# nyrahealth/CrisperWhisper

Hardware: AMD Instinct MI355X
Metric: aligned words/s (RTF alongside), CrisperWhisper large-v3 geometry, 30 s chunks, full mel->encoder->decoder->DTW->words path (higher is better)
Workload: dtype bf16

## Files before the change

### crisperwhisper_amd/csrc/engine.hip

```cpp
#include <hip/hip_runtime.h>
#include <stdarg.h>
#include <stdlib.h>
#include <string.h>
#include <set>
#include <string>
#include <vector>
#include <functional>
#include <algorithm>

#include "../../include/crisperwhisper.h"
#include "kernels.h"

static thread_local char g_err[512] = "";

#define KD(c, fn, ...) ((c)->f16 ? cw_f16::fn(__VA_ARGS__) : cw_bf16::fn(__VA_ARGS__))

#define CW_MAX_DEC_STAGES 24
enum DecStageKind { DST_OTHER = 0, DST_QKV_SELF, DST_QKV, DST_SELF_ATTN, DST_O_PROJ, DST_STACK, DST_STACK_CROSS, DST_CROSS_Q, DST_CROSS_ATTN,
                    DST_CROSS_O, DST_FC1, DST_FC2, DST_MLP_PAIR, DST_MLP_CHAIN, DST_N };
static const char* const kDecStageName[DST_N] = {
    "other (A/B path)", "LayerNorm + q/k/v projection + self-attention (qkv_self_kernel)", "LayerNorm + q/k/v projection + cache append",
    "self-attention", "self-attention out-projection", "fused out-projection + cross-query stage (gemv_stack_kernel)",
    "fused stage + cross-attention (dec_layer_a_kernel)", "LayerNorm + cross-attention query projection", "cross-attention",
    "cross-attention out-projection (combines the key-split partials)", "LayerNorm + fc1 + GELU", "fc2", "fc1 + fc2 (mlp_pair_kernel)",
// ... 2575 lines not shown
                CWCHK(c, dmalloc(c, &L.wqkv8, (size_t)3 * D * D, false)); CWCHK(c, dmalloc(c, &L.sqkv, (size_t)3 * D * 4));
                CWCHK(c, dmalloc(c, &L.w18, (size_t)F * D, false)); CWCHK(c, dmalloc(c, &L.s1, (size_t)F * 4));
                CWCHK(c, dmalloc(c, &L.w28, (size_t)D * F, false)); CWCHK(c, dmalloc(c, &L.s2, (size_t)D * 4));
            }
            for (auto& L : c->dec) { CWCHK(c, dmalloc(c, &L.wkv_c8, (size_t)2 * D * D, false)); CWCHK(c, dmalloc(c, &L.skv_c, (size_t)2 * D * 4)); }
        }
        CWCHK(c, enc8_quantise(c));
        c->enc8 = true;
        c->enc8_mask = value >= 16 ? ((value - 16) & 15) : 15;
        c->nb_encoded = 0;
        return CW_OK;
    }
#ifndef CW_EXPERIMENTS
    if ((!strcmp(name, "rows_ln") || !strcmp(name, "skinny")) && value != 0)
        return fail(c, CW_ERR_INVALID, "option %s selects a measured-and-rejected kernel variant that is not in this build (make EXTRA=-DCW_EXPERIMENTS)", name);
#endif
    if (!strcmp(name, "test_epoch_forwards")) {
        c->forwards_since_reset = (long long)value;
        return CW_OK;
    }
    if (!strcmp(name, "handoff_fail_pos")) {
        c->fail_pos = value;
        for (auto& ge : c->step_graph) if (ge) { hipGraphExecDestroy(ge); ge = nullptr; }
        return CW_OK;
    }
    if (!strcmp(name, "rows_ln")) {
        c->rows_ln_enabled = value != 0;
        for (auto& ge : c->step_graph) if (ge) { hipGraphExecDestroy(ge); ge = nullptr; }
        return CW_OK;
    }
    if (!strcmp(name, "skinny")) {
        c->skinny_mode = value;
        for (auto& ge : c->step_graph) if (ge) { hipGraphExecDestroy(ge); ge = nullptr; }
        return CW_OK;
    }
    return fail(c, CW_ERR_INVALID, "unknown option %s", name);
}

int32_t cw_has_experiments(void) {
#ifdef CW_EXPERIMENTS
    return 1;
#else
    return 0;
#endif
}

static int g_test_cross_fp8 = 0;
int32_t cw_test_set_option(const char* name, int32_t value) {
    if (!strcmp(name, "cross_test_fp8")) { g_test_cross_fp8 = value; return CW_OK; }
    if (!strcmp(name, "gemm256_min_tiles")) { cw_bf16::cw_gemm_set_256_min_tiles(value); cw_f16::cw_gemm_set_256_min_tiles(value); return CW_OK; }
    if (!strcmp(name, "beam_topk_1block")) { cw_bf16::cw_beam_topk_set_1block(value); cw_f16::cw_beam_topk_set_1block(value); return CW_OK; }
    if (!strcmp(name, "gemm_pp")) { cw_bf16::cw_gemm_set_pp(value); cw_f16::cw_gemm_set_pp(value); return CW_OK; }
    if (!strcmp(name, "gemm_8ph")) { cw_bf16::cw_gemm_set_8ph(value); cw_f16::cw_gemm_set_8ph(value); return CW_OK; }
    if (!strcmp(name, "gemm_gm")) {
#ifndef CW_EXPERIMENTS
        return CW_ERR_INVALID;
#endif
        cw_bf16::cw_gemm_set_gm(value); cw_f16::cw_gemm_set_gm(value); return CW_OK;
    }
    if (!strcmp(name, "gemv_loop")) { cw_bf16::cw_gemv_set_loop(value); cw_f16::cw_gemv_set_loop(value); return CW_OK; }
    if (!strcmp(name, "mt_variant")) { cw_bf16::cw_gemv_set_mt_variant(value); cw_f16::cw_gemv_set_mt_variant(value); return CW_OK; }
    if (!strcmp(name, "comb_rowgroups")) { cw_bf16::cw_gemv_set_comb_rowgroups(value); cw_f16::cw_gemv_set_comb_rowgroups(value); return CW_OK; }
    if (!strcmp(name, "gemm_w128")) { cw_bf16::cw_gemm_set_w128(value); cw_f16::cw_gemm_set_w128(value); return CW_OK; }
    if (!strcmp(name, "cross_valu")) { cw_bf16::cw_cross_set_valu(value); cw_f16::cw_cross_set_valu(value); return CW_OK; }
    if (!strcmp(name, "cross_per_row")) { cw_bf16::cw_cross_set_per_row(value); cw_f16::cw_cross_set_per_row(value); return CW_OK; }
    return CW_ERR_INVALID;
}

int32_t cw_test_gemm(cw_ctx* c, int32_t M, int32_t N, int32_t K, const float* A, const float* W, const float* bias,
                     int32_t gelu, float* out) {
    void *dA = nullptr, *dW = nullptr, *dO = nullptr; float* dB = nullptr;
    const size_t e = c->esz;
    HIPCHK(c, hipMalloc(&dA, (size_t)M * K * e)); HIPCHK(c, hipMalloc(&dW, (size_t)N * K * e));
    HIPCHK(c, hipMalloc(&dO, (size_t)M * N * e)); HIPCHK(c, hipMalloc((void**)&dB, (size_t)N * 4));
    CWCHK(c, upload_T(c, dA, 0, A, (size_t)M * K)); CWCHK(c, upload_T(c, dW, 0, W, (size_t)N * K));
    if (bias) HIPCHK(c, hipMemcpy(dB, bias, (size_t)N * 4, hipMemcpyHostToDevice));
    AParams ap{dA, K, 0, 0, 0, 0, nullptr, nullptr};
    EpiParams ep = epi0(); ep.out = dO; ep.bias = bias ? dB : nullptr; ep.ldo = N;
    int r = KD(c, cw_launch_gemm, c->bf16, gelu ? EPI_GELU : EPI_STORE, ap, dW, M, N, K, ep, c->st);
    if (r == CW_OK) { hipError_t er = hipStreamSynchronize(c->st); if (er != hipSuccess) r = fail(c, CW_ERR_HIP, "test_gemm: %s", hipGetErrorString(er)); }
    if (const int reps = cw_sw::cw_switches().test_gemm_reps) {
        hipEvent_t e0, e1;
        if (r == CW_OK && reps > 0 && hipEventCreate(&e0) == hipSuccess && hipEventCreate(&e1) == hipSuccess) {
            hipEventRecord(e0, c->st);
            for (int i = 0; i < reps && r == CW_OK; ++i) r = KD(c, cw_launch_gemm, c->bf16, gelu ? EPI_GELU : EPI_STORE, ap, dW, M, N, K, ep, c->st);
            hipEventRecord(e1, c->st);
            hipEventSynchronize(e1);
            float ms = 0.f;
            hipEventElapsedTime(&ms, e0, e1);
            const double us = 1e3 * ms / reps;
            fprintf(stderr, "[cw_test_gemm] M=%d N=%d K=%d gelu=%d: %.2f us/launch, %.1f TFLOP/s\n", M, N, K, gelu, us, 2.0 * M * N * K / us * 1e-6);
            hipEventDestroy(e0); hipEventDestroy(e1);
        }
    }
    if (r == CW_OK) r = download_T(c, dO, 0, out, (size_t)M * N);
    hipFree(dA); hipFree(dW); hipFree(dO); hipFree(dB);
    return r;
}

int32_t cw_test_prefill_gemm(cw_ctx* c, int32_t mode, int32_t M, int32_t N, int32_t K, const float* A, const float* W,
                             const float* bias, float* out) {
    if (!c->bf16) return fail(c, CW_ERR_INVALID, "test_prefill_gemm: 16-bit engines only");
    if ((mode != PF_STORE && mode != PF_RESID && mode != PF_GELU) || M < 1 || N < 16 || N % 16 || K < 32 || K % 32)
        return fail(c, CW_ERR_INVALID, "test_prefill_gemm: bad arguments");
    void *dA = nullptr, *dW = nullptr, *dWp = nullptr, *dO = nullptr; float* dB = nullptr;
    const size_t e = c->esz;
// ... 885 lines not shown
```

### crisperwhisper_amd/csrc/gemm.hip

```cpp
#include "common.h"
#include "kernels.h"
#include <stdlib.h>
#include <mutex>
#include "gemm_tiles.h"

namespace CW_NS {

#define BM 128
#define BN 128
#define LDS_STRIDE 72

typedef __attribute__((ext_vector_type(4))) unsigned int u32x4_t;

__device__ inline f32x4_t mfma16(bf16x8_t a, bf16x8_t b, f32x4_t c) { return cw_mfma_16x16x32(a, b, c); }

template <typename TA>
__device__ inline const TA* a_row_ptr(const AParams& ap, int m, int M, int k0) {
    if (m >= M) return nullptr;
    if (ap.amode == 0) return (const TA*)ap.A + (size_t)m * ap.lda + k0;
    int b = m / ap.T_out, t = m - b * ap.T_out;
    int tap = k0 / ap.C_in, c0 = k0 - tap * ap.C_in;
    int t_in = t * ap.stride + tap - 1;
    if (t_in < 0 || t_in >= ap.row_valid[b]) return nullptr;
    return (const TA*)ap.A + ((size_t)(ap.row_off[b] + t_in)) * ap.C_in + c0;
// ... 419 lines not shown
            asm volatile("s_waitcnt vmcnt(0)" ::: "memory");
            __builtin_amdgcn_s_barrier();
        }
        __builtin_amdgcn_s_barrier();
    } else {
        __builtin_amdgcn_s_barrier();
        for (int t = 0; t < nk; ++t) {
            read_frags(t & 1);
            if (t + 1 < nk) issue((t + 1) * BK, (t + 1) & 1);
            asm volatile("s_waitcnt vmcnt(0) lgkmcnt(0)" ::: "memory");
            __builtin_amdgcn_s_barrier();
            mfmas();
            __builtin_amdgcn_s_barrier();
        }
    }

    const bool vec_ok = (EPI == EPI_HEADS || (ep.ldo & 3) == 0);
    if (m0 + BM2 <= M && vec_ok) {
        int cols[4];
#pragma unroll
        for (int j = 0; j < 4; ++j) cols[j] = n0 + wn * 64 + j * 16 + g * 4;
#pragma unroll
        for (int h = 0; h < 2; ++h) {
            int rows[4];
#pragma unroll
            for (int i = 0; i < 4; ++i) rows[i] = m0 + wm * 128 + (h * 4 + i) * 16 + l15;
            epi_tile_interior<bf16_t, EPI>(ep, rows, cols, *(const f32x4_t(*)[4][4])&acc[h * 4]);
        }
        return;
    }
#pragma unroll
    for (int i = 0; i < 8; ++i) {
        int m = m0 + wm * 128 + i * 16 + l15;
        if (m >= M) continue;
#pragma unroll
        for (int j = 0; j < 4; ++j) {
            int n = n0 + wn * 64 + j * 16 + g * 4;
            if (vec_ok) {
                epi_store4<bf16_t, EPI>(ep, m, n, acc[i][j][0], acc[i][j][1], acc[i][j][2], acc[i][j][3]);
            } else {
#pragma unroll
                for (int r = 0; r < 4; ++r) epi_store1<bf16_t, EPI>(ep, m, n + r, acc[i][j][r]);
            }
        }
    }
}

#endif

#ifdef CW_EXPERIMENTS
__constant__ int c_gemm_gm = 8;
#endif

template <int EPI>
__global__ __launch_bounds__(512) void gemm_bf16_8ph_kernel(const bf16_t* __restrict__ A, int lda,
                                                            const bf16_t* __restrict__ W, int M, int N, int K,
                                                            EpiParams ep, int tiles_n) {
    extern __shared__ __attribute__((aligned(16))) unsigned char gsm4[];
    const int tid = threadIdx.x, lane = tid & 63;
    const int wave = __builtin_amdgcn_readfirstlane(tid >> 6);
    const int wr = wave >> 2, wn = wave & 3;
    const int l15 = lane & 15, g = lane >> 4;
#ifdef CW_EXPERIMENTS
    const int gm_ = c_gemm_gm;
    const int tile = gm_ < 0 ? (int)blockIdx.x : xcd_remap(blockIdx.x, gridDim.x);
    int mt_, nt_;
    grouped_tile(tile, gridDim.x / tiles_n, tiles_n, mt_, nt_, gm_ < 0 ? -gm_ : gm_);
#else
    const int tile = xcd_remap(blockIdx.x, gridDim.x);
    int mt_, nt_;
    grouped_tile(tile, gridDim.x / tiles_n, tiles_n, mt_, nt_);
#endif
    const int m0 = mt_ * BM2, n0 = nt_ * BN2;

    const int lrow = lane >> 3;
    const int csrc = ((lane & 7) ^ lrow) * 8;
    const __amdgpu_buffer_rsrc_t ra = __builtin_amdgcn_make_buffer_rsrc((void*)A, (short)0, 0x7fffffff, 0x00020000);
    const __amdgpu_buffer_rsrc_t rw = __builtin_amdgcn_make_buffer_rsrc((void*)W, (short)0, 0x7fffffff, 0x00020000);
    int va[2][2];
#pragma unroll
    for (int h = 0; h < 2; ++h)
#pragma unroll
        for (int q = 0; q < 2; ++q) va[h][q] = (min(m0 + h * 128 + wave * 16 + q * 8 + lrow, M - 1) * lda + csrc) * 2;
    const int vw = ((n0 + wave * 16 + lrow) * K + csrc) * 2;
    auto issue_a = [&](int k0, int buf, int h) {
#ifdef CW_8PH_NO_DMA
        return;
#endif
        unsigned char* base = gsm4 + buf * 65536 + (h * 128 + wave * 16) * 128;
#pragma unroll
        for (int q = 0; q < 2; ++q)
            __builtin_amdgcn_raw_ptr_buffer_load_lds(ra, (__attribute__((address_space(3))) void*)(base + q * 1024), 16, va[h][q], k0 * 2, 0, 0);
    };
    auto issue_w = [&](int k0, int buf, int h) {
#ifdef CW_8PH_NO_DMA
        return;
#endif
        unsigned char* base = gsm4 + buf * 65536 + 32768 + (h * 128 + wave * 16) * 128;
#pragma unroll
        for (int q = 0; q < 2; ++q)
            __builtin_amdgcn_raw_ptr_buffer_load_lds(rw, (__attribute__((address_space(3))) void*)(base + q * 1024), 16, vw,
                                                     (k0 + (h * 128 + q * 8) * K) * 2, 0, 0);
    };
    const int sw = l15 & 7;
    const int aoff = (wr * 64 + l15) * 128, woff = 32768 + (wn * 32 + l15) * 128;
    bf16x8_t fa[2][4], fw[2][2][2];
    auto read_a = [&](int buf, int h) {
#ifdef CW_8PH_NO_READS
        if (buf >= 0) return;
#endif
        const unsigned char* sb = gsm4 + buf * 65536 + aoff + h * 16384;
#pragma unroll
        for (int kk = 0; kk < 2; ++kk) {
            const int c = ((kk * 4 + g) ^ sw) << 4;
#pragma unroll
            for (int i = 0; i < 4; ++i) fa[kk][i] = *(const bf16x8_t*)(sb + i * 2048 + c);
        }
    };
    auto read_w = [&](int buf, int h) {
#ifdef CW_8PH_NO_READS
        if (buf >= 0) return;
#endif
        const unsigned char* sb = gsm4 + buf * 65536 + woff + h * 16384;
#pragma unroll
        for (int kk = 0; kk < 2; ++kk) {
            const int c = ((kk * 4 + g) ^ sw) << 4;
#pragma unroll
            for (int j = 0; j < 2; ++j) fw[h][kk][j] = *(const bf16x8_t*)(sb + j * 2048 + c);
        }
    };
    f32x4_t acc[2][4][4];
#pragma unroll
    for (int h = 0; h < 2; ++h)
#pragma unroll
        for (int i = 0; i < 4; ++i)
#pragma unroll
            for (int j = 0; j < 4; ++j) acc[h][i][j] = (f32x4_t){0.f, 0.f, 0.f, 0.f};
#define CW_8PH_COMPUTE(hm, hn)                                                                              \
    do {                                                                                                    \
        __builtin_amdgcn_s_barrier();                                                                       \
        asm volatile("s_waitcnt lgkmcnt(0)" ::: "memory");                                                  \
        __builtin_amdgcn_sched_barrier(0);                                                                  \
        __builtin_amdgcn_s_setprio(1);                                                                      \
        _Pragma("unroll") for (int kk = 0; kk < 2; ++kk)                                                    \
            _Pragma("unroll") for (int i = 0; i < 4; ++i)                                                   \
                _Pragma("unroll") for (int j = 0; j < 2; ++j)                                               \
                    acc[hm][i][(hn) * 2 + j] = mfma16(fw[hn][kk][j], fa[kk][i], acc[hm][i][(hn) * 2 + j]); \
        __builtin_amdgcn_s_setprio(0);                                                                      \
        __builtin_amdgcn_sched_barrier(0);                                                                  \
        __builtin_amdgcn_s_barrier();                                                                       \
    } while (0)
#ifndef CW_8PH_VMCNT
#define CW_8PH_VMCNT 6
#endif
#define CW_8PH_STR2(x) #x
#define CW_8PH_STR(x) CW_8PH_STR2(x)
#define CW_8PH_WAIT(steady)                                                                                 \
    do {                                                                                                    \
        if (steady) asm volatile("s_waitcnt vmcnt(" CW_8PH_STR(CW_8PH_VMCNT) ")" ::: "memory");             \
        else asm volatile("s_waitcnt vmcnt(0)" ::: "memory");                                               \
        __builtin_amdgcn_sched_barrier(0);                                                                  \
    } while (0)

    const int nk = K / BK;
    issue_a(0, 0, 0); issue_w(0, 0, 0); issue_w(0, 0, 1); issue_a(0, 0, 1);
    if (nk > 1) issue_a(BK, 1, 0);
    asm volatile("s_waitcnt vmcnt(0)" ::: "memory");
    __builtin_amdgcn_s_barrier();
    if (wr == 1) __builtin_amdgcn_s_barrier();
    for (int t = 0; t < nk; ++t) {
        const int b = t & 1, nb = b ^ 1;
        const bool nxt = t + 1 < nk, nxt2 = t + 2 < nk;
        const bool steady = t + 2 < nk;
        const int k1 = (t + 1) * BK, k2 = (t + 2) * BK;
        read_w(b, 0);
        __builtin_amdgcn_sched_barrier(0);
        read_a(b, 0);
        __builtin_amdgcn_sched_barrier(0);
        if (nxt) issue_w(k1, nb, 0);
        CW_8PH_WAIT(steady);
        CW_8PH_COMPUTE(0, 0);
        read_w(b, 1);
        __builtin_amdgcn_sched_barrier(0);
        if (nxt) issue_w(k1, nb, 1);
        CW_8PH_WAIT(steady);
        CW_8PH_COMPUTE(0, 1);
        read_a(b, 1);
        __builtin_amdgcn_sched_barrier(0);
        if (nxt) issue_a(k1, nb, 1);
        CW_8PH_WAIT(steady);
        CW_8PH_COMPUTE(1, 1);
        if (nxt2) issue_a(k2, b, 0);
        CW_8PH_WAIT(steady);
        CW_8PH_COMPUTE(1, 0);
    }
    if (wr == 0) __builtin_amdgcn_s_barrier();
#undef CW_8PH_COMPUTE
#undef CW_8PH_WAIT

    const bool vec_ok = (EPI == EPI_HEADS || (ep.ldo & 3) == 0);
    int cols[4];
#pragma unroll
    for (int j = 0; j < 4; ++j) cols[j] = n0 + (j >> 1) * 128 + wn * 32 + (j & 1) * 16 + g * 4;
    if (m0 + BM2 <= M && vec_ok) {
#pragma unroll
        for (int h = 0; h < 2; ++h) {
            int rows[4];
#pragma unroll
            for (int i = 0; i < 4; ++i) rows[i] = m0 + h * 128 + wr * 64 + i * 16 + l15;
            epi_tile_interior<bf16_t, EPI>(ep, rows, cols, acc[h]);
        }
        return;
    }
#pragma unroll
    for (int h = 0; h < 2; ++h)
#pragma unroll
        for (int i = 0; i < 4; ++i) {
            const int m = m0 + h * 128 + wr * 64 + i * 16 + l15;
            if (m >= M) continue;
#pragma unroll
            for (int j = 0; j < 4; ++j) {
                const int n = cols[j];
                if (vec_ok) {
                    epi_store4<bf16_t, EPI>(ep, m, n, acc[h][i][j][0], acc[h][i][j][1], acc[h][i][j][2], acc[h][i][j][3]);
                } else {
#pragma unroll
                    for (int r = 0; r < 4; ++r) epi_store1<bf16_t, EPI>(ep, m, n + r, acc[h][i][j][r]);
                }
            }
        }
}

typedef __attribute__((ext_vector_type(8))) int i32x8_t;
__device__ inline i32x8_t frag_fp8(const unsigned char* row, int c_lo, int c_hi) {
    const u32x4_t lo = *(const u32x4_t*)(row + c_lo), hi = *(const u32x4_t*)(row + c_hi);
    return (i32x8_t){(int)lo[0], (int)lo[1], (int)lo[2], (int)lo[3], (int)hi[0], (int)hi[1], (int)hi[2], (int)hi[3]};
}

template <int EPI>
__global__ __launch_bounds__(512) void gemm_fp8_pp_kernel(const unsigned char* __restrict__ A, int lda,
                                                          const unsigned char* __restrict__ W, int M, int N, int K,
                                                          const float* __restrict__ sa, const float* __restrict__ sw,
                                                          EpiParams ep, int tiles_n) {
    extern __shared__ __attribute__((aligned(16))) unsigned char gsm4[];
    const int tid = threadIdx.x, lane = tid & 63;
    const int wave = __builtin_amdgcn_readfirstlane(tid >> 6);
    const int wm = wave >> 2, wn = wave & 3;
    const int l15 = lane & 15, g = lane >> 4;
    const int tile = xcd_remap(blockIdx.x, gridDim.x);
    int mt_, nt_;
    grouped_tile(tile, gridDim.x / tiles_n, tiles_n, mt_, nt_);
    const int m0 = mt_ * BM2, n0 = nt_ * BN2;

    const int lrow = lane >> 3;
    const int csrc = ((lane & 7) ^ lrow) * 16;
    const __amdgpu_buffer_rsrc_t ra = __builtin_amdgcn_make_buffer_rsrc((void*)A, (short)0, 0x7fffffff, 0x00020000);
    const __amdgpu_buffer_rsrc_t rw = __builtin_amdgcn_make_buffer_rsrc((void*)W, (short)0, 0x7fffffff, 0x00020000);
    int va[4];
#pragma unroll
    for (int q = 0; q < 4; ++q) va[q] = min(m0 + wave * 32 + q * 8 + lrow, M - 1) * lda + csrc;
    const int vw = (n0 + wave * 32 + lrow) * K + csrc;
    auto issue = [&](int k0, int buf) {
        unsigned char* base = gsm4 + buf * 65536 + wave * 4096;
#pragma unroll
        for (int q = 0; q < 4; ++q) {
            __builtin_amdgcn_raw_ptr_buffer_load_lds(ra, (__attribute__((address_space(3))) void*)(base + q * 1024), 16, va[q], k0, 0, 0);
            __builtin_amdgcn_raw_ptr_buffer_load_lds(rw, (__attribute__((address_space(3))) void*)(base + 32768 + q * 1024), 16, vw,
                                                     k0 + q * 8 * K, 0, 0);
        }
    };
    const int sw_ = l15 & 7;
    const int aoff = (wm * 128 + l15) * 128, woff = 32768 + (wn * 64 + l15) * 128;
    i32x8_t fa[8], fw[4];
    const int c_lo = (g ^ sw_) << 4, c_hi = ((4 + g) ^ sw_) << 4;
    auto read_frags = [&](int buf) {
        const unsigned char* sb = gsm4 + buf * 65536;
#pragma unroll
        for (int j = 0; j < 4; ++j) fw[j] = frag_fp8(sb + woff + j * 2048, c_lo, c_hi);
#pragma unroll
        for (int i = 0; i < 8; ++i) fa[i] = frag_fp8(sb + aoff + i * 2048, c_lo, c_hi);
    };
    f32x4_t acc[8][4];
#pragma unroll
// ... 886 lines not shown
                    ex.xf_out[frag_index(m, n[c], ep.ldo)] = f32_to_bf16(y);
                    s1 += y; s2 += y * y;
                } else {
                    EpiParams e2 = ep;
                    e2.bias = nullptr;
                    if (EPI == EPI_QKV_CACHE) { e2.row_pos = nullptr; e2.row_pos_pre = rpos_pre[t]; }
                    epi_store1<bf16_t, EPI>(e2, m, n[c], EPI == EPI_RESID_F32 ? resid_grid(v + bias_v[c]) : v + bias_v[c]);
                }
            }
        }
        if (MODE2 == 1) {
#pragma unroll
            for (int msk = 1; msk < 16; msk <<= 1) { s1 += __shfl_xor(s1, msk, 64); s2 += __shfl_xor(s2, msk, 64); }
            if (l15 == 0 && m < Mb) {
                float* so = ex.stats_out + ((size_t)blockIdx.x * 64 + m) * 2;
                so[0] = s1; so[1] = s2;
            }
        }
    }
}

template <int EPI>
__global__ __launch_bounds__(256) void gemv_f32_kernel(const float* __restrict__ x, int Mb, int K,
                                                       const float* __restrict__ W, int N, EpiParams ep) {
    const int lane = threadIdx.x & 63, wave = threadIdx.x >> 6;
    const int n = blockIdx.x * 4 + wave;
    if (n >= N) return;
    const float* wr = W + (size_t)n * K;
    for (int mb = 0; mb < Mb; mb += 8) {
        float acc[8] = {};
        for (int k = lane; k < K; k += 64) {
            float w = wr[k];
#pragma unroll
            for (int i = 0; i < 8; ++i)
                if (mb + i < Mb) acc[i] = fmaf(x[(size_t)(mb + i) * K + k], w, acc[i]);
        }
#pragma unroll
        for (int i = 0; i < 8; ++i) {
            float v = wave_sum(acc[i]);
            if (lane == 0 && mb + i < Mb) epi_store1<float, EPI>(ep, mb + i, n, v);
        }
    }
}

static const bf16_t* g_zero_page = nullptr;
static bool g_use_glds = true;
static bool g_use_256 = true;
static int g_256_min_tiles = 200;
static int g_use_pp = -1;
void cw_gemm_set_256_min_tiles(int n) { g_256_min_tiles = n; }
static int g_use_8ph = -1;
void cw_gemm_set_pp(int on) { g_use_pp = on; }
void cw_gemm_set_8ph(int on) { g_use_8ph = on; }
void cw_gemm_set_gm(int gm) {
#ifdef CW_EXPERIMENTS
    if (gm == 0) gm = 8;
    (void)hipMemcpyToSymbol(HIP_SYMBOL(c_gemm_gm), &gm, sizeof(int));
#else
    (void)gm;
#endif
}
static int g_gemv_loop = -1;
void cw_gemv_set_loop(int on) { g_gemv_loop = on; }
static int g_comb_rowgroups = -1;
void cw_gemv_set_comb_rowgroups(int on) { g_comb_rowgroups = on; }
static int g_use_w128 = -1;
void cw_gemm_set_w128(int on) { g_use_w128 = on; }

template <int EPI>
static void launch_gemm_epi(bool bf16, const AParams& ap, const void* W, int M, int N, int K, const EpiParams& ep,
                            hipStream_t st) {
    if (bf16) {
        int tm = (M + BM - 1) / BM, tn = (N + BN - 1) / BN;
        static std::once_flag once;
        std::call_once(once, [] {
            void* z = nullptr;
            if (hipMalloc(&z, 256) == hipSuccess) { hipMemset(z, 0, 256); g_zero_page = (const bf16_t*)z; }
            if (cw_sw::cw_switches().no_glds) g_use_glds = false;
            if (cw_sw::cw_switches().no_gemm256) g_use_256 = false;
        });
        const int tm2 = (M + BM2 - 1) / BM2, tn2 = (N + BN2 - 1) / BN2;
        if (g_use_pp < 0) g_use_pp = !cw_sw::cw_switches().no_gemm_pp;
        const bool use_pp = g_use_pp != 0;
        if (g_use_8ph < 0) g_use_8ph = !cw_sw::cw_switches().no_gemm_8ph;
#ifdef CW_EXPERIMENTS
        if (g_use_w128 < 0) g_use_w128 = cw_sw::cw_switches().gemm_w128;
#else
        g_use_w128 = 0;
#endif
        if (g_use_glds && g_zero_page && g_use_256 && g_use_w128 && tm2 * tn2 >= g_256_min_tiles && ap.amode == 0 && N % BN2 == 0) {
            cw_launch_gemm_w128(EPI, (const bf16_t*)ap.A, ap.lda, (const bf16_t*)W, M, N, K, ep, tm2, tn2, st);
        } else if (g_use_glds && g_zero_page && g_use_256 && use_pp && g_use_8ph && tm2 * tn2 >= g_256_min_tiles && ap.amode == 0 && N % BN2 == 0) {
            static std::once_flag attr_8;
            std::call_once(attr_8, [] {
                hipFuncSetAttribute((const void*)gemm_bf16_8ph_kernel<EPI>, hipFuncAttributeMaxDynamicSharedMemorySize, 131072);
            });
            hipLaunchKernelGGL((gemm_bf16_8ph_kernel<EPI>), dim3(tm2 * tn2), dim3(512), 131072, st, (const bf16_t*)ap.A, ap.lda,
                               (const bf16_t*)W, M, N, K, ep, tn2);
#ifdef CW_EXPERIMENTS
        } else if (g_use_glds && g_zero_page && g_use_256 && use_pp && tm2 * tn2 >= g_256_min_tiles && ap.amode == 0 && N % BN2 == 0) {
            static std::once_flag attr_pp;
            std::call_once(attr_pp, [] {
                hipFuncSetAttribute((const void*)gemm_bf16_pp_kernel<EPI>, hipFuncAttributeMaxDynamicSharedMemorySize, 131072);
            });
            hipLaunchKernelGGL((gemm_bf16_pp_kernel<EPI>), dim3(tm2 * tn2), dim3(512), 131072, st, (const bf16_t*)ap.A, ap.lda,
                               (const bf16_t*)W, M, N, K, ep, tn2, g_zero_page);
#endif
        } else if (g_use_glds && g_zero_page && g_use_256 && tm2 * tn2 >= g_256_min_tiles) {
            static std::once_flag attr_once;
            std::call_once(attr_once, [] {
                hipFuncSetAttribute((const void*)gemm_bf16_256_kernel<EPI>, hipFuncAttributeMaxDynamicSharedMemorySize, 131072);
            });
            hipLaunchKernelGGL((gemm_bf16_256_kernel<EPI>), dim3(tm2 * tn2), dim3(512), 131072, st, ap, (const bf16_t*)W, M,
                               N, K, ep, tn2, g_zero_page);
        } else if (g_use_glds && g_zero_page)
            hipLaunchKernelGGL((gemm_bf16_glds_kernel<EPI>), dim3(tm * tn), dim3(256), 65536, st, ap, (const bf16_t*)W, M,
                               N, K, ep, tn, g_zero_page);
        else
        hipLaunchKernelGGL((gemm_bf16_kernel<EPI>), dim3(tm * tn), dim3(256), 0, st, ap, (const bf16_t*)W, M, N, K, ep,
                           tn);
    } else {
        int tm = (M + 63) / 64, tn = (N + 63) / 64;
        hipLaunchKernelGGL((gemm_f32_kernel<EPI>), dim3(tm * tn), dim3(256), 0, st, ap, (const float*)W, M, N, K, ep,
                           tn);
    }
}

int cw_launch_gemm(bool bf16, int epi, const AParams& ap, const void* W, int M, int N, int K, const EpiParams& ep,
                   hipStream_t st) {
    if (K % 64 != 0 || M <= 0 || N <= 0) return CW_ERR_INVALID;
    switch (epi) {
        case EPI_STORE: launch_gemm_epi<EPI_STORE>(bf16, ap, W, M, N, K, ep, st); break;
        case EPI_GELU: launch_gemm_epi<EPI_GELU>(bf16, ap, W, M, N, K, ep, st); break;
        case EPI_RESID_F32: launch_gemm_epi<EPI_RESID_F32>(bf16, ap, W, M, N, K, ep, st); break;
        case EPI_GELU_POS_F32: launch_gemm_epi<EPI_GELU_POS_F32>(bf16, ap, W, M, N, K, ep, st); break;
        case EPI_HEADS: launch_gemm_epi<EPI_HEADS>(bf16, ap, W, M, N, K, ep, st); break;
        case EPI_STORE_F32: launch_gemm_epi<EPI_STORE_F32>(bf16, ap, W, M, N, K, ep, st); break;
        default: return CW_ERR_INVALID;
    }
    return CW_OK;
}

int cw_launch_quant_rows_fp8(const void* x, int rows, int K, void* out8, float* scale, hipStream_t st) {
    if (K % 8 != 0 || rows <= 0) return CW_ERR_INVALID;
    hipLaunchKernelGGL(quant_rows_fp8_kernel, dim3((rows + 3) / 4), dim3(256), 0, st, (const bf16_t*)x, rows, K, (unsigned char*)out8, scale);
    return CW_OK;
}

template <int EPI>
static void launch_gemm_fp8_epi(const void* A8, int lda, const void* W8, int M, int N, int K, const float* sa, const float* sw,
                                const EpiParams& ep, hipStream_t st) {
// ... 364 lines not shown
```

### crisperwhisper_amd/csrc/kernels.h

```cpp
#pragma once
#include "switches.h"
#include "common.h"

struct AParams {
    const void* A;
    int lda;
    int amode;
    int T_out, C_in, stride;
    const int* row_off;
    const int* row_valid;
};

struct CombineParams;


struct SampleParams {
    const float* logits;
    int V, B, ldv;
    const unsigned char* mask;
    int eos, pad, timestamp_begin, max_initial_timestamp_index;
    const int* cfg;
    int* pos;
    int ids_stride;
    int* ids;
// ... 219 lines not shown
    const void* W1;
    const float* b1;
    const void* W2;
    const float* b2;
    float* xio;
    void* mid;
    unsigned long long* flags;
    const unsigned int* epoch;
    int layer;
    int* err;
    int Mb, D, F;
    int Kb2;
    int delay;
};

struct MelTables {
    const double* cos_t;
    const double* sin_t;
    const double* window;
    const float* filters;
    const int* fb_lo;
    const int* fb_hi;
    int dbg;
};


enum PrefillMode { PF_STORE = 0, PF_QKV = 1, PF_RESID = 2, PF_GELU = 3 };
struct PrefillEpi {
    int mode;
    const float* bias;
    void* out;
    float* x;
    void* sk; void* sv;
    int D, H, cap, n_pos;
};
struct PrefillAlign {
    float* out;
    float* ml;
    const int* slot;
    int n_align, rows;
};

struct ScorePart {
    float mx, sum;
    float tl;
    float bv; int bi;
};

#define CW_DTYPE_KERNEL_DECLS \
    int cw_launch_gemm(bool bf16, int epi, const AParams& ap, const void* W, int M, int N, int K, const EpiParams& ep, hipStream_t st); \
    void cw_gemm_set_256_min_tiles(int n); \
    void cw_gemm_set_pp(int on); \
    void cw_gemm_set_8ph(int on); \
    void cw_gemm_set_gm(int gm); \
    void cw_gemm_set_w128(int on); \
    void cw_gemv_set_comb_rowgroups(int on); \
    void cw_gemv_set_mt_variant(int v); \
    void cw_gemv_set_loop(int on); \
    int cw_launch_gemm_w128(int epi, const bf16_t* A, int lda, const bf16_t* W, int M, int N, int K, const EpiParams& ep, int tm2, int tn2, hipStream_t st); \
    void cw_cross_set_valu(int on); \
    void cw_cross_set_per_row(int on); \
    int cw_launch_layernorm_fp8(const float* x, const float* g, const float* b, void* out8, float* scale, int rows, int d, hipStream_t st); \
    int cw_launch_quant_rows_fp8(const void* x, int rows, int K, void* out8, float* scale, hipStream_t st); \
    int cw_launch_gemm_fp8(int epi, const void* A8, int lda, const void* W8, int M, int N, int K, const float* sa, const float* sw, const EpiParams& ep, hipStream_t st); \
    int cw_launch_fold_layernorm(const float* Wf, int N, int K, const float* g, const float* beta, float scale, void* w_out, float* bias, hipStream_t st); \
    int cw_launch_gemv(bool bf16, int epi, const float* x, int Mb, int K, const void* W, int N, const float* ln_g, const float* ln_b, const EpiParams& ep, hipStream_t st, const CombineParams* comb = nullptr, void* scratch = nullptr, bool wpacked = false); \
    int cw_gemv_own_nt(int N); \
    int cw_launch_gemv_own(const void* xf, int Mb, int K, const void* W, int N, const EpiParams& ep, const float* cvec, void* xf_out, float* stats_out, hipStream_t st, bool wpacked); \
    int cw_launch_gemv_lna(const void* xf, int Mb, int K, const void* W, int N, const EpiParams& ep, const float* stats_in, int n_stats, const float* wsum, hipStream_t st, bool wpacked); \
    size_t cw_wfrag_elems(int N, int K); \
    int cw_launch_wfrag_pack(const void* src, int N, int K, void* dst, hipStream_t st); \
    int cw_launch_fold_product(const float* A, const float* s, float scale, const float* B, int N, int J, int K, void* C16, hipStream_t st); \
    int cw_launch_fold_rowvec(const float* A, const float* s, float scale, const float* v, const void* W16, int N, int J, float* c_out, float* w_out, hipStream_t st); \
    int cw_launch_gemv_stack(const StackParams& p, int nt, hipStream_t st); \
    int cw_launch_dec_layer(const DecLayerParams& p, int n_cu, hipStream_t st); \
    bool cw_mlp_chain_ok(int Mb, int D, int F); \
    int cw_launch_mlp_chain(const MlpChainParams& p, hipStream_t st); \
    int cw_launch_qkv_self(const QkvSelfParams& p, hipStream_t st); \
    int cw_qkv_self_blocks_per_cu(int D, int cap); \
    size_t cw_dec_layer_lds(int D); \
    int cw_launch_gemv_fc2x(const Fc2xParams& p, hipStream_t st); \
    int cw_launch_mlp_pair(const MlpPairParams& p, hipStream_t st); \
    int cw_launch_gemv_rows(int epi, bool produce, const RowsParams& p, hipStream_t st); \
    int cw_launch_rows_combine(const float* part_o, int Mb, int K, const CombineParams& cb, void* xf, hipStream_t st); \
    int cw_launch_rows_prep(const float* x, int Mb, int K, void* xf, float* pstats, int lo_off, hipStream_t st); \
    int cw_skinny_pick_nks(int N, int K, int s_max); \
    int cw_launch_skinny(int mode, const SkinnyParams& p, int nks, hipStream_t st); \
    int cw_launch_skinny_finish(int epi, const SkinnyFinishParams& p, hipStream_t st); \
    void cw_launch_skinny_empty(hipStream_t st); \
    int cw_launch_layernorm(bool bf16_out, const float* x, const float* g, const float* b, void* out, int rows, int d, hipStream_t st); \
    int cw_launch_layernorm_f32(const float* x, const float* g, const float* b, float* out, int rows, int d, hipStream_t st); \
    int cw_launch_sample(const SampleParams& p, hipStream_t st); \
    int cw_launch_beam_topk(const SampleParams& p, int n_cand, float* cand_val, int* cand_id, float* scratch, hipStream_t st); \
    size_t cw_beam_topk_scratch_floats(int rows); \
    void cw_beam_topk_set_1block(int on); \
    int cw_launch_beam_advance(const BeamAdvanceParams& p, hipStream_t st); \
    int cw_launch_align_gather(const float* align, const int* row_of_pos, int n_items, int n_align, int align_rows, int L, int n_keys, float* out, hipStream_t st); \
    int cw_launch_set_pos(int* pos, int value, int B, hipStream_t st, unsigned int* epoch = nullptr); \
    int cw_launch_embed(const int* ids, int ids_stride, int t, const void* embed, int embed_bf16, const float* pos_embed, float* x_out, int B, int d, hipStream_t st); \
    int cw_launch_prefill_embed(const int* ids, int ids_stride, int n_pos, const void* embed, const float* pos_embed, float* x, int M, int D, hipStream_t st); \
    int cw_launch_prefill_ln(const float* x, void* out, int M, int D, hipStream_t st); \
    int cw_launch_prefill_gemm(const void* A, const void* W, const PrefillEpi& ep, int M, int N, int K, hipStream_t st); \
    int cw_launch_prefill_attn(const void* Q, const void* K, const void* V, void* out, int rows, int n_q, int H, int cap, int n_keys, int causal, int kv_div, hipStream_t st); \
    int cw_launch_prefill_attn_align(const void* Q, const void* K, const void* V, void* out, int rows, int n_q, int H, int cap, int n_keys, int causal, int kv_div, const PrefillAlign& al, hipStream_t st); \
    int cw_launch_score_ln(const float* x, const int* src, const float* g, const float* b, void* out, int M, int D, hipStream_t st); \
    int cw_score_head_splits(int M, int V, int* tiles_per_split); \
// ... 30 lines not shown
```

### crisperwhisper_amd/csrc/switches.cpp

```cpp
#include "switches.h"
#include <cstdlib>

namespace cw_sw {

static bool flag(const char* name) { return getenv(name) != nullptr; }
static int num(const char* name, int dflt) { const char* v = getenv(name); return v ? atoi(v) : dflt; }

Switches read_switches() {
    Switches s{};
    s.no_graph = flag("CW_NO_GRAPH");
    s.no_ln_fold = flag("CW_NO_LN_FOLD");
    s.no_fuse6 = flag("CW_NO_FUSE6");
    s.rows_ln = flag("CW_ROWS_LN");
    s.no_rows_hilo = flag("CW_NO_ROWS_HILO");
    s.no_stack_center = flag("CW_NO_STACK_CENTER");
    s.no_mid16 = flag("CW_NO_MID16");
    s.dtw_block = flag("CW_DTW_BLOCK");
    s.fuse_mlp = flag("CW_FUSE_MLP");
    s.no_wpack = flag("CW_NO_WPACK");
    s.mlp_pair = flag("CW_MLP_PAIR");
    s.mlp_pair_fence = flag("CW_MLP_PAIR_FENCE");
    s.declayer = flag("CW_DECLAYER");
    s.no_qkv_self = flag("CW_NO_QKV_SELF");
    s.mlp_chain = flag("CW_MLP_CHAIN");
    s.no_fuse_rows = flag("CW_NO_FUSE_ROWS");
    s.no_fuse_rows8 = flag("CW_NO_FUSE_ROWS8");
    s.no_fuse_beam = flag("CW_NO_FUSE_BEAM");
    s.no_own_cols = flag("CW_NO_OWN_COLS");
    s.no_short_hist = flag("CW_NO_SHORT_HIST");
    s.skinny = num("CW_SKINNY", 0);
    s.prefetch = num("CW_PREFETCH", 0);
    s.prefetch_wide = num("CW_PREFETCH_WIDE", 0);
    s.prefetch_what = num("CW_PREFETCH_WHAT", 3);
    s.stack_nt3 = num("CW_STACK_NT3", 0);
    s.stack_nt5 = num("CW_STACK_NT5", 0);
    s.attn_v1 = flag("CW_ATTN_V1");
    s.anc_attn_v1 = flag("CW_ANC_ATTN_V1");
    s.cross_per_row = flag("CW_CROSS_PER_ROW");
    s.cross_valu = flag("CW_CROSS_VALU");
    s.cross_no_tr = flag("CW_CROSS_NO_TR");
    s.cross8_valu = flag("CW_CROSS8_VALU");
    s.cross_mfma1 = flag("CW_CROSS_MFMA1");
    s.cross_lds_pad = num("CW_CROSS_LDS_PAD", 0);
    s.cross8_nsb = num("CW_CROSS8_NSB", 0);
    s.dl_depth = num("CW_DL_DEPTH", 16);
    s.dl_kvwait = num("CW_DL_KVWAIT", 0);
    s.mlp_chain_delay = num("CW_MLP_CHAIN_DELAY", 0);
    s.qkv_self_dbg = num("CW_QKV_SELF_DBG", 0);
    s.no_glds = flag("CW_NO_GLDS");
    s.no_gemm256 = flag("CW_NO_GEMM256");
    s.no_gemm_pp = flag("CW_NO_GEMM_PP");
    s.no_gemm_8ph = flag("CW_NO_GEMM_8PH");
    s.gemm_w128 = flag("CW_GEMM_W128");
    s.no_gemv_loop = flag("CW_NO_GEMV_LOOP");
    s.comb_nt2 = flag("CW_COMB_NT2");
    s.comb_no_rowgroups = flag("CW_COMB_NO_ROWGROUPS");
    s.comb_g4 = flag("CW_COMB_G4");
    s.mt_no_prea = flag("CW_MT_NO_PREA");
    s.gemv_loop_cap = num("CW_GEMV_LOOP_CAP", 512);
    s.fc2_ksplit = num("CW_FC2_KSPLIT", 0);
    s.mt_variant = num("CW_MT_VARIANT", -1);
    s.own_nt = num("CW_OWN_NT", 1);
    if (s.mt_variant < -1 || s.mt_variant > 2) s.mt_variant = -1;
    s.beam_topk_1block = flag("CW_BEAM_TOPK_1BLOCK");
    s.mel_valu = flag("CW_MEL_VALU");
    s.mel_dbg = num("CW_MEL_DBG", 0);
    s.test_gemm_reps = num("CW_TEST_GEMM_REPS", 0);
    s.test_attn_reps = num("CW_TEST_ATTN_REPS", 0);
    if (s.gemv_loop_cap < 1) s.gemv_loop_cap = 1;
    if (s.fc2_ksplit < 0) s.fc2_ksplit = 0;
    if (s.cross_lds_pad < 0) s.cross_lds_pad = 0;
    if (s.cross_lds_pad > 150 * 1024) s.cross_lds_pad = 150 * 1024;
    if (s.stack_nt3 < 0 || s.stack_nt3 > 3) s.stack_nt3 = 0;
    if (s.stack_nt5 < 0 || s.stack_nt5 > 3) s.stack_nt5 = 0;
    if (s.prefetch < 0) s.prefetch = 0;
    if (s.mlp_chain_delay < 0 || s.mlp_chain_delay > 4096) s.mlp_chain_delay = 0;
    if (s.test_gemm_reps < 0) s.test_gemm_reps = 0;
    if (s.test_attn_reps < 0) s.test_attn_reps = 0;
    return s;
}

const Switches& cw_switches() {
    static const Switches s = read_switches();
    return s;
}

}
```

### crisperwhisper_amd/csrc/switches.h

```cpp
#pragma once

namespace cw_sw {

struct Switches {
    bool no_graph, no_ln_fold, no_fuse6, rows_ln, no_rows_hilo, no_stack_center, no_mid16, dtw_block, fuse_mlp, no_wpack, mlp_pair, mlp_pair_fence, declayer, no_qkv_self, mlp_chain, no_fuse_rows, no_fuse_rows8, no_fuse_beam, no_own_cols, no_short_hist;
    int skinny, prefetch, prefetch_wide, prefetch_what, stack_nt3, stack_nt5;
    bool attn_v1, anc_attn_v1, cross_per_row, cross_valu, cross_no_tr, cross8_valu, cross_mfma1;
    int cross_lds_pad, cross8_nsb, dl_depth, dl_kvwait, mlp_chain_delay, qkv_self_dbg;
    bool no_glds, no_gemm256, no_gemm_pp, no_gemm_8ph, gemm_w128, no_gemv_loop, comb_nt2, comb_no_rowgroups, mt_no_prea, comb_g4;
    int gemv_loop_cap, fc2_ksplit, mt_variant, own_nt;
    bool beam_topk_1block, mel_valu;
    int mel_dbg;
    int test_gemm_reps, test_attn_reps;
};

const Switches& cw_switches();
Switches read_switches();

}
```

Measured before the change: 760.0.

## Add persistent-grid mode to 8-phase GEMM, overlapping next tile prologue with epilogue

The 8-phase bf16 GEMM can now run as a persistent kernel. When there are more tiles than CUs, the grid is capped at the CU count and each block loops over tiles. Before writing the current tile's epilogue, it computes the next tile's coordinates and issues that tile's first LDS DMA loads, so those loads overlap the stores. The aim is to cut per-block launch and ramp-up cost and fix wave-quantization tails on encoder GEMMs. The cost is a static schedule that loses dynamic load balancing, the risk of LDS-reuse hazards between the prologue DMA and the epilogue, and extra register pressure from the loop.

After: 760.6, median of 5. About the same (+0.1%).

```diff
diff --git a/crisperwhisper_amd/csrc/engine.hip b/crisperwhisper_amd/csrc/engine.hip
--- a/crisperwhisper_amd/csrc/engine.hip
+++ b/crisperwhisper_amd/csrc/engine.hip
@@ -2651,6 +2651,11 @@
     if (!strcmp(name, "beam_topk_1block")) { cw_bf16::cw_beam_topk_set_1block(value); cw_f16::cw_beam_topk_set_1block(value); return CW_OK; }
     if (!strcmp(name, "gemm_pp")) { cw_bf16::cw_gemm_set_pp(value); cw_f16::cw_gemm_set_pp(value); return CW_OK; }
     if (!strcmp(name, "gemm_8ph")) { cw_bf16::cw_gemm_set_8ph(value); cw_f16::cw_gemm_set_8ph(value); return CW_OK; }
+    if (!strcmp(name, "gemm_persist")) { cw_bf16::cw_gemm_set_persist(value); cw_f16::cw_gemm_set_persist(value); return CW_OK; }
+    if (!strcmp(name, "gemm_persist_blocks")) {
+        if (value < 0) return CW_ERR_INVALID;
+        cw_bf16::cw_gemm_set_persist_blocks(value); cw_f16::cw_gemm_set_persist_blocks(value); return CW_OK;
+    }
     if (!strcmp(name, "gemm_gm")) {
 #ifndef CW_EXPERIMENTS
         return CW_ERR_INVALID;
diff --git a/crisperwhisper_amd/csrc/gemm.hip b/crisperwhisper_amd/csrc/gemm.hip
--- a/crisperwhisper_amd/csrc/gemm.hip
+++ b/crisperwhisper_amd/csrc/gemm.hip
@@ -495,37 +495,46 @@
 __constant__ int c_gemm_gm = 8;
 #endif
 
-template <int EPI>
+template <int EPI, int PERSIST>
 __global__ __launch_bounds__(512) void gemm_bf16_8ph_kernel(const bf16_t* __restrict__ A, int lda,
                                                             const bf16_t* __restrict__ W, int M, int N, int K,
-                                                            EpiParams ep, int tiles_n) {
+                                                            EpiParams ep, int tiles_n, int n_tiles) {
     extern __shared__ __attribute__((aligned(16))) unsigned char gsm4[];
     const int tid = threadIdx.x, lane = tid & 63;
     const int wave = __builtin_amdgcn_readfirstlane(tid >> 6);
     const int wr = wave >> 2, wn = wave & 3;
     const int l15 = lane & 15, g = lane >> 4;
+    const int total = PERSIST ? n_tiles : (int)gridDim.x;
+    int m0, n0;
+    auto locate = [&](int idx) {
 #ifdef CW_EXPERIMENTS
-    const int gm_ = c_gemm_gm;
-    const int tile = gm_ < 0 ? (int)blockIdx.x : xcd_remap(blockIdx.x, gridDim.x);
-    int mt_, nt_;
-    grouped_tile(tile, gridDim.x / tiles_n, tiles_n, mt_, nt_, gm_ < 0 ? -gm_ : gm_);
+        const int gm_ = c_gemm_gm;
+        const int tile = gm_ < 0 ? idx : xcd_remap(idx, total);
+        int mt_, nt_;
+        grouped_tile(tile, total / tiles_n, tiles_n, mt_, nt_, gm_ < 0 ? -gm_ : gm_);
 #else
-    const int tile = xcd_remap(blockIdx.x, gridDim.x);
-    int mt_, nt_;
-    grouped_tile(tile, gridDim.x / tiles_n, tiles_n, mt_, nt_);
+        const int tile = xcd_remap(idx, total);
+        int mt_, nt_;
+        grouped_tile(tile, total / tiles_n, tiles_n, mt_, nt_);
 #endif
-    const int m0 = mt_ * BM2, n0 = nt_ * BN2;
+        m0 = mt_ * BM2; n0 = nt_ * BN2;
+    };
+    int idx = blockIdx.x;
+    locate(idx);
 
     const int lrow = lane >> 3;
     const int csrc = ((lane & 7) ^ lrow) * 8;
     const __amdgpu_buffer_rsrc_t ra = __builtin_amdgcn_make_buffer_rsrc((void*)A, (short)0, 0x7fffffff, 0x00020000);
     const __amdgpu_buffer_rsrc_t rw = __builtin_amdgcn_make_buffer_rsrc((void*)W, (short)0, 0x7fffffff, 0x00020000);
-    int va[2][2];
-#pragma unroll
-    for (int h = 0; h < 2; ++h)
-#pragma unroll
-        for (int q = 0; q < 2; ++q) va[h][q] = (min(m0 + h * 128 + wave * 16 + q * 8 + lrow, M - 1) * lda + csrc) * 2;
-    const int vw = ((n0 + wave * 16 + lrow) * K + csrc) * 2;
+    int va[2][2], vw;
+    auto aim = [&]() {
+#pragma unroll
+        for (int h = 0; h < 2; ++h)
+#pragma unroll
+            for (int q = 0; q < 2; ++q) va[h][q] = (min(m0 + h * 128 + wave * 16 + q * 8 + lrow, M - 1) * lda + csrc) * 2;
+        vw = ((n0 + wave * 16 + lrow) * K + csrc) * 2;
+    };
+    aim();
     auto issue_a = [&](int k0, int buf, int h) {
 #ifdef CW_8PH_NO_DMA
         return;
@@ -605,73 +614,100 @@
         __builtin_amdgcn_sched_barrier(0);                                                                  \
     } while (0)
 
+    auto epilogue = [&](const EpiParams& e, int em0, int en0) {
+        const bool vec_ok = (EPI == EPI_HEADS || (e.ldo & 3) == 0);
+        int cols[4];
+#pragma unroll
+        for (int j = 0; j < 4; ++j) cols[j] = en0 + (j >> 1) * 128 + wn * 32 + (j & 1) * 16 + g * 4;
+        if (em0 + BM2 <= M && vec_ok) {
+#pragma unroll
+            for (int h = 0; h < 2; ++h) {
+                int rows[4];
+#pragma unroll
+                for (int i = 0; i < 4; ++i) rows[i] = em0 + h * 128 + wr * 64 + i * 16 + l15;
+                epi_tile_interior<bf16_t, EPI>(e, rows, cols, acc[h]);
+            }
+            return;
+        }
+#pragma unroll
+        for (int h = 0; h < 2; ++h)
+#pragma unroll
+            for (int i = 0; i < 4; ++i) {
+                const int m = em0 + h * 128 + wr * 64 + i * 16 + l15;
+                if (m >= M) continue;
+#pragma unroll
+                for (int j = 0; j < 4; ++j) {
+                    const int n = cols[j];
+                    if (vec_ok) {
+                        epi_store4<bf16_t, EPI>(e, m, n, acc[h][i][j][0], acc[h][i][j][1], acc[h][i][j][2], acc[h][i][j][3]);
+                    } else {
+#pragma unroll
+                        for (int r = 0; r < 4; ++r) epi_store1<bf16_t, EPI>(e, m, n + r, acc[h][i][j][r]);
+                    }
+                }
+            }
+    };
     const int nk = K / BK;
-    issue_a(0, 0, 0); issue_w(0, 0, 0); issue_w(0, 0, 1); issue_a(0, 0, 1);
-    if (nk > 1) issue_a(BK, 1, 0);
-    asm volatile("s_waitcnt vmcnt(0)" ::: "memory");
-    __builtin_amdgcn_s_barrier();
-    if (wr == 1) __builtin_amdgcn_s_barrier();
-    for (int t = 0; t < nk; ++t) {
-        const int b = t & 1, nb = b ^ 1;
-        const bool nxt = t + 1 < nk, nxt2 = t + 2 < nk;
-        const bool steady = t + 2 < nk;
-        const int k1 = (t + 1) * BK, k2 = (t + 2) * BK;
-        read_w(b, 0);
-        __builtin_amdgcn_sched_barrier(0);
-        read_a(b, 0);
-        __builtin_amdgcn_sched_barrier(0);
-        if (nxt) issue_w(k1, nb, 0);
-        CW_8PH_WAIT(steady);
-        CW_8PH_COMPUTE(0, 0);
-        read_w(b, 1);
-        __builtin_amdgcn_sched_barrier(0);
-        if (nxt) issue_w(k1, nb, 1);
-        CW_8PH_WAIT(steady);
-        CW_8PH_COMPUTE(0, 1);
-        read_a(b, 1);
-        __builtin_amdgcn_sched_barrier(0);
-        if (nxt) issue_a(k1, nb, 1);
-        CW_8PH_WAIT(steady);
-        CW_8PH_COMPUTE(1, 1);
-        if (nxt2) issue_a(k2, b, 0);
-        CW_8PH_WAIT(steady);
-        CW_8PH_COMPUTE(1, 0);
-    }
-    if (wr == 0) __builtin_amdgcn_s_barrier();
+    auto issue_prologue = [&]() {
+        issue_a(0, 0, 0); issue_w(0, 0, 0); issue_w(0, 0, 1); issue_a(0, 0, 1);
+        if (nk > 1) issue_a(BK, 1, 0);
+    };
+    issue_prologue();
+    for (;;) {
+        asm volatile("s_waitcnt vmcnt(0)" ::: "memory");
+        __builtin_amdgcn_s_barrier();
+        if (wr == 1) __builtin_amdgcn_s_barrier();
+        for (int t = 0; t < nk; ++t) {
+            const int b = t & 1, nb = b ^ 1;
+            const bool nxt = t + 1 < nk, nxt2 = t + 2 < nk;
+            const bool steady = t + 2 < nk;
+            const int k1 = (t + 1) * BK, k2 = (t + 2) * BK;
+            read_w(b, 0);
+            __builtin_amdgcn_sched_barrier(0);
+            read_a(b, 0);
+            __builtin_amdgcn_sched_barrier(0);
+            if (nxt) issue_w(k1, nb, 0);
+            CW_8PH_WAIT(steady);
+            CW_8PH_COMPUTE(0, 0);
+            read_w(b, 1);
+            __builtin_amdgcn_sched_barrier(0);
+            if (nxt) issue_w(k1, nb, 1);
+            CW_8PH_WAIT(steady);
+            CW_8PH_COMPUTE(0, 1);
+            read_a(b, 1);
+            __builtin_amdgcn_sched_barrier(0);
+            if (nxt) issue_a(k1, nb, 1);
+            CW_8PH_WAIT(steady);
+            CW_8PH_COMPUTE(1, 1);
+            if (nxt2) issue_a(k2, b, 0);
+            CW_8PH_WAIT(steady);
+            CW_8PH_COMPUTE(1, 0);
+        }
+        if (wr == 0) __builtin_amdgcn_s_barrier();
+        if (!PERSIST) {
+            epilogue(ep, m0, n0);
+            return;
+        }
+        const int em0 = m0, en0 = n0;
+        idx += gridDim.x;
+        const bool more = idx < total;
+        if (more) {
+            locate(idx);
+            aim();
+            issue_prologue();
+            __builtin_amdgcn_sched_barrier(0);
+        }
+        epilogue(ep, em0, en0);
+        if (!more) return;
+#pragma unroll
+        for (int h = 0; h < 2; ++h)
+#pragma unroll
+            for (int i = 0; i < 4; ++i)
+#pragma unroll
+                for (int j = 0; j < 4; ++j) acc[h][i][j] = (f32x4_t){0.f, 0.f, 0.f, 0.f};
+    }
 #undef CW_8PH_COMPUTE
 #undef CW_8PH_WAIT
-
-    const bool vec_ok = (EPI == EPI_HEADS || (ep.ldo & 3) == 0);
-    int cols[4];
-#pragma unroll
-    for (int j = 0; j < 4; ++j) cols[j] = n0 + (j >> 1) * 128 + wn * 32 + (j & 1) * 16 + g * 4;
-    if (m0 + BM2 <= M && vec_ok) {
-#pragma unroll
-        for (int h = 0; h < 2; ++h) {
-            int rows[4];
-#pragma unroll
-            for (int i = 0; i < 4; ++i) rows[i] = m0 + h * 128 + wr * 64 + i * 16 + l15;
-            epi_tile_interior<bf16_t, EPI>(ep, rows, cols, acc[h]);
-        }
-        return;
-    }
-#pragma unroll
-    for (int h = 0; h < 2; ++h)
-#pragma unroll
-        for (int i = 0; i < 4; ++i) {
-            const int m = m0 + h * 128 + wr * 64 + i * 16 + l15;
-            if (m >= M) continue;
-#pragma unroll
-            for (int j = 0; j < 4; ++j) {
-                const int n = cols[j];
-                if (vec_ok) {
-                    epi_store4<bf16_t, EPI>(ep, m, n, acc[h][i][j][0], acc[h][i][j][1], acc[h][i][j][2], acc[h][i][j][3]);
-                } else {
-#pragma unroll
-                    for (int r = 0; r < 4; ++r) epi_store1<bf16_t, EPI>(ep, m, n + r, acc[h][i][j][r]);
-                }
-            }
-        }
 }
 
 typedef __attribute__((ext_vector_type(8))) int i32x8_t;
@@ -1664,6 +1700,22 @@
 static int g_use_8ph = -1;
 void cw_gemm_set_pp(int on) { g_use_pp = on; }
 void cw_gemm_set_8ph(int on) { g_use_8ph = on; }
+static int g_use_persist = -1;
+static int g_persist_blocks = 0;
+static int g_n_cu = 0;
+void cw_gemm_set_persist(int on) { g_use_persist = on; }
+void cw_gemm_set_persist_blocks(int n) { g_persist_blocks = n; }
+static int persist_grid(int n_tiles) {
+    if (g_use_persist < 0) g_use_persist = !cw_sw::cw_switches().no_gemm_persist;
+    if (!g_use_persist) return 0;
+    if (g_n_cu == 0) {
+        int dev = 0, n = 0;
+        if (hipGetDevice(&dev) == hipSuccess && hipDeviceGetAttribute(&n, hipDeviceAttributeMultiprocessorCount, dev) == hipSuccess) g_n_cu = n;
+        if (g_n_cu < 1) g_n_cu = 256;
+    }
+    const int cap = g_persist_blocks > 0 ? g_persist_blocks : g_n_cu;
+    return n_tiles > cap ? cap : 0;
+}
 void cw_gemm_set_gm(int gm) {
 #ifdef CW_EXPERIMENTS
     if (gm == 0) gm = 8;
@@ -1705,10 +1757,15 @@
         } else if (g_use_glds && g_zero_page && g_use_256 && use_pp && g_use_8ph && tm2 * tn2 >= g_256_min_tiles && ap.amode == 0 && N % BN2 == 0) {
             static std::once_flag attr_8;
             std::call_once(attr_8, [] {
-                hipFuncSetAttribute((const void*)gemm_bf16_8ph_kernel<EPI>, hipFuncAttributeMaxDynamicSharedMemorySize, 131072);
+                hipFuncSetAttribute((const void*)gemm_bf16_8ph_kernel<EPI, 0>, hipFuncAttributeMaxDynamicSharedMemorySize, 131072);
+                hipFuncSetAttribute((const void*)gemm_bf16_8ph_kernel<EPI, 1>, hipFuncAttributeMaxDynamicSharedMemorySize, 131072);
             });
-            hipLaunchKernelGGL((gemm_bf16_8ph_kernel<EPI>), dim3(tm2 * tn2), dim3(512), 131072, st, (const bf16_t*)ap.A, ap.lda,
-                               (const bf16_t*)W, M, N, K, ep, tn2);
+            if (const int pg = persist_grid(tm2 * tn2))
+                hipLaunchKernelGGL((gemm_bf16_8ph_kernel<EPI, 1>), dim3(pg), dim3(512), 131072, st, (const bf16_t*)ap.A, ap.lda,
+                                   (const bf16_t*)W, M, N, K, ep, tn2, tm2 * tn2);
+            else
+            hipLaunchKernelGGL((gemm_bf16_8ph_kernel<EPI, 0>), dim3(tm2 * tn2), dim3(512), 131072, st, (const bf16_t*)ap.A, ap.lda,
+                               (const bf16_t*)W, M, N, K, ep, tn2, tm2 * tn2);
 #ifdef CW_EXPERIMENTS
         } else if (g_use_glds && g_zero_page && g_use_256 && use_pp && tm2 * tn2 >= g_256_min_tiles && ap.amode == 0 && N % BN2 == 0) {
             static std::once_flag attr_pp;
diff --git a/crisperwhisper_amd/csrc/kernels.h b/crisperwhisper_amd/csrc/kernels.h
--- a/crisperwhisper_amd/csrc/kernels.h
+++ b/crisperwhisper_amd/csrc/kernels.h
@@ -295,6 +295,8 @@
     void cw_gemm_set_256_min_tiles(int n); \
     void cw_gemm_set_pp(int on); \
     void cw_gemm_set_8ph(int on); \
+    void cw_gemm_set_persist(int on); \
+    void cw_gemm_set_persist_blocks(int n); \
     void cw_gemm_set_gm(int gm); \
     void cw_gemm_set_w128(int on); \
     void cw_gemv_set_comb_rowgroups(int on); \
diff --git a/crisperwhisper_amd/csrc/switches.cpp b/crisperwhisper_amd/csrc/switches.cpp
--- a/crisperwhisper_amd/csrc/switches.cpp
+++ b/crisperwhisper_amd/csrc/switches.cpp
@@ -51,6 +51,7 @@
     s.no_gemm256 = flag("CW_NO_GEMM256");
     s.no_gemm_pp = flag("CW_NO_GEMM_PP");
     s.no_gemm_8ph = flag("CW_NO_GEMM_8PH");
+    s.no_gemm_persist = flag("CW_NO_GEMM_PERSIST");
     s.gemm_w128 = flag("CW_GEMM_W128");
     s.no_gemv_loop = flag("CW_NO_GEMV_LOOP");
     s.comb_nt2 = flag("CW_COMB_NT2");
diff --git a/crisperwhisper_amd/csrc/switches.h b/crisperwhisper_amd/csrc/switches.h
--- a/crisperwhisper_amd/csrc/switches.h
+++ b/crisperwhisper_amd/csrc/switches.h
@@ -7,7 +7,7 @@
     int skinny, prefetch, prefetch_wide, prefetch_what, stack_nt3, stack_nt5;
     bool attn_v1, anc_attn_v1, cross_per_row, cross_valu, cross_no_tr, cross8_valu, cross_mfma1;
     int cross_lds_pad, cross8_nsb, dl_depth, dl_kvwait, mlp_chain_delay, qkv_self_dbg;
-    bool no_glds, no_gemm256, no_gemm_pp, no_gemm_8ph, gemm_w128, no_gemv_loop, comb_nt2, comb_no_rowgroups, mt_no_prea, comb_g4;
+    bool no_glds, no_gemm256, no_gemm_pp, no_gemm_8ph, no_gemm_persist, gemm_w128, no_gemv_loop, comb_nt2, comb_no_rowgroups, mt_no_prea, comb_g4;
     int gemv_loop_cap, fc2_ksplit, mt_variant, own_nt;
     bool beam_topk_1block, mel_valu;
     int mel_dbg;
```
